# MarSaKi/VLN-BEVBert

Hardware: AMD Instinct MI355X
Metric: pretrain_samples_per_sec (higher is better)
Workload: dtype bf16+fp32-residual

## Files before the change

include/bevbert_hip.h:

```cpp
#ifndef BEVBERT_HIP_H
#define BEVBERT_HIP_H

#include <stdint.h>

#ifdef __cplusplus
extern "C" {
#endif

typedef struct ihipStream_t* hipStream_t;

#define BEVBERT_F32 0
#define BEVBERT_BF16 1
#define BEVBERT_F16 2

const char* bevbert_last_error(void);
int bevbert_version(void);
int bevbert_hip_error_reset(void);
const char* bevbert_arch(void);
const char* bevbert_attn_last_path(int backward);
const char* bevbert_attn_plan(int B, int nh, int Lq, int Lk, int dtype, int impl, int has_key_mask, int has_bias,
                              float drop_p, int has_bits, int bits_ready, int want_dbias, int ncu, int backward);

int bevbert_bev_lift_bin(const float* depths, const float* T_c2w, const float* T_w2c, const float* S_w2c,
                         const float* pix_scale, int B, int V, int hw, float depth_scale, int dim, float res,
                         float y_clip, int* cell, int* order, int* cell_start, hipStream_t stream);
int bevbert_bev_bin_points(const float* points, const uint8_t* drop_mask, int B, int P, int dim, float res,
                           float y_clip, int* cell, int* order, int* cell_start, hipStream_t stream);
int bevbert_bev_splat_mean(const void* feat, int feat_dtype, const int* order, const int* cell_start, void* out,
                           int out_dtype, int B, int P, int K, int C, const uint8_t* sem_ids, const double* sem_dense,
                           int S, uint8_t* out_sem, uint8_t* out_sem_mask, const int* sample_rows, int rows_per_sample,
                           hipStream_t stream);

int bevbert_attn_fwd(const void* q, const void* k, const void* v, void* o, float* lse, const float* key_mask,
                     const float* bias, const int64_t* strides, int B, int nh, int Lq, int Lk, int head_dim,
                     float scale, int dtype, int impl, float drop_p, uint64_t seed, uint64_t offset,
                     uint64_t* drop_bits, int bits_ready, hipStream_t stream);
int bevbert_attn_bwd(const void* q, const void* k, const void* v, const void* o, const void* dout, const float* lse,
                     float* delta_ws, void* dq, void* dk, void* dv, float* dbias, const float* key_mask,
                     const float* bias, const int64_t* strides, int B, int nh, int Lq, int Lk, int head_dim,
                     float scale, int dtype, int impl, float drop_p, uint64_t seed, uint64_t offset,
                     const uint64_t* drop_bits, hipStream_t stream);
int64_t bevbert_attn_drop_bits_words(int B, int nh, int Lq, int Lk);
int bevbert_attn_drop_bits(uint64_t* drop_bits, int B, int nh, int Lq, int Lk, float drop_p, uint64_t seed,
                           uint64_t offset, hipStream_t stream);
int bevbert_attn_bits_ahead(int Lq, int Lk, int has_bias);

int bevbert_bias_dropout_residual_layernorm_fwd(const void* x, const float* bias, const void* residual,
                                                const float* gamma, const float* beta, void* y, void* z_out,
                                                float* mean, float* rstd, int rows, int H, float eps, int dtype,
                                                float drop_p, uint64_t seed, uint64_t offset, hipStream_t stream);
int bevbert_layernorm_post_fwd(const void* x, const float* bias, const float* gamma, const float* beta,
                               const void* post1, const void* post2, void* y, void* z_out, float* mean, float* rstd,
                               int rows, int H, float eps, int dtype, hipStream_t stream);
int bevbert_layernorm_bwd(const void* dy, const void* z, const float* mean, const float* rstd, const float* gamma,
// ... 204 lines not shown
```

vln_bevbert_amd/csrc/capi.hip:

```cpp
#include <stdarg.h>

#include "attn_common.h"

static thread_local char g_err[512] = "";

void bb_set_error(const char* fmt, ...) {
  va_list ap;
  va_start(ap, fmt);
  vsnprintf(g_err, sizeof(g_err), fmt, ap);
  va_end(ap);
}

BEVBERT_API const char* bevbert_last_error(void) { return g_err; }
BEVBERT_API int bevbert_hip_error_reset(void) {
  int n = 0;
  while (hipGetLastError() != hipSuccess && n < 16) ++n;
  return n;
}

BEVBERT_API int bevbert_zero(void* p, int64_t bytes, hipStream_t stream) {
  BB_REQUIRE(p != nullptr && bytes >= 0, "zero: null pointer or negative size");
  if (bytes == 0) return BB_OK;
  hipError_t e = hipMemsetAsync(p, 0, (size_t)bytes, stream);
  if (e != hipSuccess) {
    bb_set_error("zero: hipMemsetAsync failed: %s", hipGetErrorString(e));
    return BB_ELAUNCH;
  }
  return BB_OK;
}

BEVBERT_API int bevbert_version(void) { return 201; }

static const uint32_t* g_step_salt = nullptr;
const uint32_t* bb_step_salt() { return g_step_salt; }
BEVBERT_API int bevbert_set_step_salt(const void* device_word) {
  g_step_salt = static_cast<const uint32_t*>(device_word);
  return BB_OK;
}
BEVBERT_API const char* bevbert_arch(void) { return "gfx950"; }

int attn_simple_fwd(const AttnArgs& a, int dtype, hipStream_t st);
int attn_simple_bwd(const AttnArgs& a, int dtype, hipStream_t st);
int attn_delta(const AttnArgs& a, float* delta, int dtype, hipStream_t st);
int attn_mfma_fwd(const AttnArgs& a, hipStream_t st);
int attn_mfma_bwd(const AttnArgs& a, hipStream_t st);
int attn_mfma_bwd1(const AttnArgs& a, hipStream_t st);
bool attn_mfma_bwd1_supported(const AttnArgs& a);
int attn_fwd2(const AttnArgs& a, hipStream_t st);
bool attn_fwd2_supported(const AttnArgs& a);
int attn_drop_bits(const AttnArgs& a, uint64_t* bits_f, uint64_t* bits_b, uint32_t* bits_l, hipStream_t st);
int attn_fwd4(const AttnArgs& a, const uint32_t* bits_l, hipStream_t st);
bool attn_fwd4_supported(const AttnArgs& a, int ncu, bool forced);
int attn_fwd4_workgroups();
int attn_bwd2(const AttnArgs& a, hipStream_t st);
// ... 256 lines not shown
```

vln_bevbert_amd/csrc/splat.hip:

```cpp
#include "common.h"

#define MAX_CELLS 1024
#define MAX_POINTS 24576

struct LiftArgs {
  const float* depths;
  const float* T_c2w;
  const float* T_w2c;
  const float* S_w2c;
  const float* pix;
  const float* points;
  const uint8_t* pmask;
  int V, hw;
  float depth_scale;
  int P, dim;
  float res, half, y_clip;
  int* cell;
  int* order;
  int* cell_start;
};

__device__ __forceinline__ int cell_of(float ex, float ey, float ez, bool dropped, int dim, float res, float half,
                                       float y_clip) {
  const float fx = rintf(__fadd_rn(__fdiv_rn(ex, res), half));
  const float fz = rintf(__fadd_rn(__fdiv_rn(ez, res), half));
  const float fd = (float)dim;
  const bool outside = (fx >= fd) | (fz >= fd) | (fx < 0.f) | (fz < 0.f);
  if (dropped | outside | (ey > y_clip)) return -1;
  return dim * (int)fz + (int)fx;
}

template <int MODE>
__global__ __launch_bounds__(256) void bev_bin_sort_kernel(LiftArgs a) {
  __shared__ short s_cell[MAX_POINTS];
  __shared__ int s_cnt[MAX_CELLS + 1];
  const int b = blockIdx.x, tid = threadIdx.x;
  const int K = a.dim * a.dim;
  for (int c = tid; c <= K; c += 256) s_cnt[c] = 0;
  __syncthreads();

  for (int p = tid; p < a.P; p += 256) {
    int cid;
    if (MODE == 0) {
      const int hw2 = a.hw * a.hw;
      const int v = p / hw2, r = (p - v * hw2) / a.hw, u = p % a.hw;
      const float z = __fmul_rn(a.depths[(size_t)b * a.P + p], a.depth_scale);
      const float x = __fmul_rn(z, a.pix[u]);
      const float y = __fmul_rn(z, a.pix[r]);
      const float* T = a.T_c2w + ((size_t)b * a.V + v) * 16;
      float w[3];
#pragma unroll
      for (int i = 0; i < 3; ++i)
        w[i] = __fadd_rn(__fadd_rn(__fadd_rn(__fmul_rn(T[i * 4 + 0], x), __fmul_rn(T[i * 4 + 1], y)),
                                   __fmul_rn(T[i * 4 + 2], z)),
                         T[i * 4 + 3]);
      const float* S = a.S_w2c + (size_t)b * 3;
      const float p0 = __fsub_rn(w[0], S[0]), p1 = __fsub_rn(w[1], S[1]), p2 = __fsub_rn(w[2], S[2]);
      const float* R = a.T_w2c + (size_t)b * 16;
      float e[3];
#pragma unroll
      for (int i = 0; i < 3; ++i)
        e[i] = __fadd_rn(__fadd_rn(__fadd_rn(__fmul_rn(R[i * 4 + 0], p0), __fmul_rn(R[i * 4 + 1], p1)),
                                   __fmul_rn(R[i * 4 + 2], p2)),
                         R[i * 4 + 3]);
      cid = cell_of(e[0], e[1], e[2], z == 0.f, a.dim, a.res, a.half, a.y_clip);
    } else {
      const float* q = a.points + ((size_t)b * a.P + p) * 3;
      cid = cell_of(q[0], q[1], q[2], a.pmask[(size_t)b * a.P + p] != 0, a.dim, a.res, a.half, a.y_clip);
    }
    s_cell[p] = (short)cid;
    a.cell[(size_t)b * a.P + p] = cid;
    if (cid >= 0) atomicAdd(&s_cnt[cid], 1);
  }
  __syncthreads();

  if (tid < 64) {
    const int per = (K + 63) / 64;
    const int c0 = tid * per;
    int sum = 0;
    for (int i = 0; i < per; ++i)
      if (c0 + i < K) sum += s_cnt[c0 + i];
    int incl = sum;
#pragma unroll
    for (int o = 1; o < 64; o <<= 1) {
      int t = __shfl_up(incl, o, 64);
      if (tid >= o) incl += t;
    }
    int run = incl - sum;
    for (int i = 0; i < per; ++i)
      if (c0 + i < K) {
        const int n = s_cnt[c0 + i];
        s_cnt[c0 + i] = run;
        run += n;
      }
    if (tid == 63) s_cnt[K] = incl;
  }
  __syncthreads();
  for (int c = tid; c <= K; c += 256) a.cell_start[(size_t)b * (K + 1) + c] = s_cnt[c];

  __shared__ int s_wbase[4][MAX_CELLS + 1];
  const int lane = tid & 63, wv = tid >> 6;
  for (int c = tid; c < 4 * (MAX_CELLS + 1); c += 256) (&s_wbase[0][0])[c] = 0;
  __syncthreads();
  const int per_wave = ((a.P + 255) / 256) * 64;
  const int pw0 = wv * per_wave;
  for (int p = pw0 + lane; p < pw0 + per_wave && p < a.P; p += 64) {
    const int cid = s_cell[p];
    if (cid >= 0) atomicAdd(&s_wbase[wv][cid], 1);
  }
  __syncthreads();
  for (int c = tid; c < K; c += 256) {
    int base = s_cnt[c];
#pragma unroll
    for (int w = 0; w < 4; ++w) {
      const int n = s_wbase[w][c];
      s_wbase[w][c] = base;
      base += n;
    }
  }
  __syncthreads();
  int* dst = a.order + (size_t)b * a.P;
  const unsigned long long lt = lane == 0 ? 0ull : (~0ull >> (64 - lane));
  for (int p0 = pw0; p0 < pw0 + per_wave && p0 < a.P; p0 += 64) {
    const int p = p0 + lane;
    const int cid = p < a.P ? (int)s_cell[p] : -1;
    unsigned long long todo = __ballot(cid >= 0);
    while (todo) {
      const int leader = __builtin_ctzll(todo);
      const int c0 = __shfl(cid, leader, 64);
      const unsigned long long same = __ballot(cid == c0);
      const int base = s_wbase[wv][c0];
      if (cid == c0) dst[base + __builtin_popcountll(same & lt)] = p;
      if (lane == leader) s_wbase[wv][c0] = base + __builtin_popcountll(same);
      todo &= ~same;
    }
  }
}

template <typename TI, typename TO>
__global__ __launch_bounds__(256) void bev_splat_mean_kernel(const TI* __restrict__ feat, const int* __restrict__ order,
                                                             const int* __restrict__ cell_start, TO* __restrict__ out,
                                                             int P, int K, int C,
                                                             const uint8_t* __restrict__ sem_ids,
                                                             const double* __restrict__ sem_dense,
                                                             int S, uint8_t* __restrict__ out_sem,
                                                             uint8_t* __restrict__ out_sem_mask,
                                                             const int* __restrict__ sample_rows,
                                                             int R) {
  const int cellg = blockIdx.x;
  const int b = cellg / K, cell = cellg - b * K;
  const int P0 = P / R;
  const int* rows = sample_rows != nullptr ? sample_rows + (size_t)b * R : nullptr;
  auto src_point = [&](int p) -> size_t {
    if (rows == nullptr) return (size_t)b * P + p;
    if (R == 1) return (size_t)rows[0] * P0 + p;
    const int r = p / P0;
    return (size_t)rows[r] * P0 + (p - r * P0);
  };
  const int s0 = cell_start[(size_t)b * (K + 1) + cell];
  const int n = cell_start[(size_t)b * (K + 1) + cell + 1] - s0;
  const int* ord = order + (size_t)b * P + s0;
  const float inv_denominator = (float)(n > 1 ? n : 1);

  for (int c4 = threadIdx.x; c4 * 4 < C; c4 += blockDim.x) {
    float4 acc = make_float4(0.f, 0.f, 0.f, 0.f);
    int i = 0;
    for (; i + 4 <= n; i += 4) {
      const int p0 = ord[i], p1 = ord[i + 1], p2 = ord[i + 2], p3 = ord[i + 3];
      const float4 v0 = ld4<TI>(feat + src_point(p0) * C + c4 * 4);
      const float4 v1 = ld4<TI>(feat + src_point(p1) * C + c4 * 4);
      const float4 v2 = ld4<TI>(feat + src_point(p2) * C + c4 * 4);
      const float4 v3 = ld4<TI>(feat + src_point(p3) * C + c4 * 4);
      acc.x = __fadd_rn(__fadd_rn(__fadd_rn(__fadd_rn(acc.x, v0.x), v1.x), v2.x), v3.x);
      acc.y = __fadd_rn(__fadd_rn(__fadd_rn(__fadd_rn(acc.y, v0.y), v1.y), v2.y), v3.y);
      acc.z = __fadd_rn(__fadd_rn(__fadd_rn(__fadd_rn(acc.z, v0.z), v1.z), v2.z), v3.z);
      acc.w = __fadd_rn(__fadd_rn(__fadd_rn(__fadd_rn(acc.w, v0.w), v1.w), v2.w), v3.w);
    }
    for (; i < n; ++i) {
      const float4 v = ld4<TI>(feat + src_point(ord[i]) * C + c4 * 4);
      acc.x = __fadd_rn(acc.x, v.x); acc.y = __fadd_rn(acc.y, v.y);
      acc.z = __fadd_rn(acc.z, v.z); acc.w = __fadd_rn(acc.w, v.w);
    }
    acc.x = __fdiv_rn(acc.x, inv_denominator); acc.y = __fdiv_rn(acc.y, inv_denominator);
    acc.z = __fdiv_rn(acc.z, inv_denominator); acc.w = __fdiv_rn(acc.w, inv_denominator);
    st4<TO>(out + (size_t)cellg * C + c4 * 4, acc);
  }

  if (out_sem != nullptr) {
    int any = 0;
    for (int c = threadIdx.x; c < S; c += blockDim.x) {
      uint8_t flag = 0;
      if (sem_ids != nullptr) {
        for (int i = 0; i < n; ++i) flag |= (uint8_t)(sem_ids[src_point(ord[i])] == (uint8_t)c);
      } else {
        const double* sb = sem_dense + (size_t)b * P * S;
        double acc = 0.0;
        for (int i = 0; i < n; ++i) acc += sb[(size_t)ord[i] * S + c];
        flag = (uint8_t)(acc / (double)(n > 1 ? n : 1) > 0.0);
      }
      out_sem[(size_t)cellg * S + c] = flag;
      any |= flag;
    }
    any = __syncthreads_or(any);
    if (threadIdx.x == 0) out_sem_mask[cellg] = (uint8_t)(any != 0);
  }
}

BEVBERT_API int bevbert_bev_lift_bin(const float* depths, const float* T_c2w, const float* T_w2c, const float* S_w2c,
                                     const float* pix_scale, int B, int V, int hw, float depth_scale, int dim,
                                     float res, float y_clip, int* cell, int* order, int* cell_start,
                                     hipStream_t stream) {
  const int P = V * hw * hw;
  BB_REQUIRE(B > 0 && P > 0 && P <= MAX_POINTS, "bev_lift_bin: P=%d out of range (max %d)", P, MAX_POINTS);
  BB_REQUIRE(dim > 0 && dim * dim <= MAX_CELLS, "bev_lift_bin: dim=%d too large", dim);
  LiftArgs a;
  memset(&a, 0, sizeof(a));
  a.depths = depths; a.T_c2w = T_c2w; a.T_w2c = T_w2c; a.S_w2c = S_w2c; a.pix = pix_scale;
  a.V = V; a.hw = hw; a.depth_scale = depth_scale; a.P = P; a.dim = dim; a.res = res;
  a.half = (float)(dim - 1) / 2.0f; a.y_clip = y_clip;
  a.cell = cell; a.order = order; a.cell_start = cell_start;
  hipLaunchKernelGGL(bev_bin_sort_kernel<0>, dim3(B), dim3(256), 0, stream, a);
  BB_CHECK_LAUNCH("bev_lift_bin");
  return BB_OK;
}

BEVBERT_API int bevbert_bev_bin_points(const float* points, const uint8_t* drop_mask, int B, int P, int dim, float res,
                                       float y_clip, int* cell, int* order, int* cell_start, hipStream_t stream) {
  BB_REQUIRE(B > 0 && P > 0 && P <= MAX_POINTS, "bev_bin_points: P=%d out of range (max %d)", P, MAX_POINTS);
  BB_REQUIRE(dim > 0 && dim * dim <= MAX_CELLS, "bev_bin_points: dim=%d too large", dim);
  LiftArgs a;
  memset(&a, 0, sizeof(a));
  a.points = points; a.pmask = drop_mask; a.P = P; a.dim = dim; a.res = res;
  a.half = (float)(dim - 1) / 2.0f; a.y_clip = y_clip;
  a.cell = cell; a.order = order; a.cell_start = cell_start;
  hipLaunchKernelGGL(bev_bin_sort_kernel<1>, dim3(B), dim3(256), 0, stream, a);
  BB_CHECK_LAUNCH("bev_bin_points");
  return BB_OK;
}

template <typename TI, typename TO>
static int launch_splat(const void* feat, const int* order, const int* cell_start, void* out, int B, int P, int K,
                        int C, const uint8_t* sem_ids, const double* sem_dense, int S, uint8_t* out_sem,
                        uint8_t* out_sem_mask, const int* sample_rows, int R, hipStream_t stream) {
  const int threads = (C / 4 >= 192) ? 192 : ((C / 4 + 63) / 64) * 64;
  hipLaunchKernelGGL((bev_splat_mean_kernel<TI, TO>), dim3(B * K), dim3(threads < 64 ? 64 : threads), 0, stream,
                     (const TI*)feat, order, cell_start, (TO*)out, P, K, C, sem_ids, sem_dense, S, out_sem,
                     out_sem_mask, sample_rows, R);
  BB_CHECK_LAUNCH("bev_splat_mean");
  return BB_OK;
}

BEVBERT_API int bevbert_bev_splat_mean(const void* feat, int feat_dtype, const int* order, const int* cell_start,
                                       void* out, int out_dtype, int B, int P, int K, int C, const uint8_t* sem_ids,
                                       const double* sem_dense, int S, uint8_t* out_sem, uint8_t* out_sem_mask,
                                       const int* sample_rows, int rows_per_sample, hipStream_t stream) {
  BB_REQUIRE(C % 4 == 0, "bev_splat_mean: C=%d must be a multiple of 4", C);
  const int R = rows_per_sample < 1 ? 1 : rows_per_sample;
  BB_REQUIRE(R == 1 || sample_rows != nullptr, "bev_splat_mean: rows_per_sample=%d needs sample_rows", R);
  BB_REQUIRE(P % R == 0, "bev_splat_mean: P=%d is not a multiple of rows_per_sample=%d", P, R);
  BB_REQUIRE(sample_rows == nullptr || sem_dense == nullptr,
             "bev_splat_mean: sample_rows indexes feat / sem_ids stores; dense semantics are per batch");
  BB_REQUIRE(out_sem == nullptr || (sem_ids != nullptr) != (sem_dense != nullptr),
             "bev_splat_mean: exactly one of sem_ids / sem_dense when semantics are requested");
#define GO(TI, TO) \
  return launch_splat<TI, TO>(feat, order, cell_start, out, B, P, K, C, sem_ids, sem_dense, S, out_sem, out_sem_mask, sample_rows, R, stream)
  if (feat_dtype == BB_F32 && out_dtype == BB_F32) GO(float, float);
  if (feat_dtype == BB_F32 && out_dtype == BB_BF16) GO(float, bf16_raw);
  if (feat_dtype == BB_BF16 && out_dtype == BB_F32) GO(bf16_raw, float);
  if (feat_dtype == BB_BF16 && out_dtype == BB_BF16) GO(bf16_raw, bf16_raw);
  if (feat_dtype == BB_F16 && out_dtype == BB_F32) GO(_Float16, float);
  if (feat_dtype == BB_F16 && out_dtype == BB_BF16) GO(_Float16, bf16_raw);
  if (feat_dtype == BB_F16 && out_dtype == BB_F16) GO(_Float16, _Float16);
#undef GO
  bb_set_error("bev_splat_mean: unsupported dtype pair (%d -> %d)", feat_dtype, out_dtype);
  return BB_EUNSUPPORTED;
}
```

vln_bevbert_amd/lib.py:

```python
import ctypes
import os
import re
import subprocess

import torch

_HERE = os.path.dirname(os.path.abspath(__file__))
LIB_PATH = os.path.join(_HERE, "libbevbert_hip.so")
CSRC = os.path.join(_HERE, "csrc")
EXTRA_FLAGS = {"attn_fwd4.hip": ["-fno-slp-vectorize"]}
SOURCES = ["splat.hip", "rowops.hip", "attn_simple.hip", "attn_f32.hip", "attn_mfma.hip", "attn_bwd1.hip", "attn_fwd2.hip", "attn_fwd4.hip", "attn_bwd2.hip", "attn_bwd3.hip", "attn_small.hip", "attn_short.hip", "smallk.hip", "sap_loss.hip", "graph_nav.hip", "nav_expert.hip", "waypoint.hip", "gemm.hip", "capi.hip"]
HEADER = os.path.join(os.path.dirname(_HERE), "include", "bevbert_hip.h")

F32, BF16, F16 = 0, 1, 2
_DT = {torch.float32: F32, torch.bfloat16: BF16, torch.float16: F16}


class BevBertHipError(RuntimeError):
    pass


def dtype_code(t):
    try:
        return _DT[t.dtype if torch.is_tensor(t) else t]
# ... 21 lines not shown
    def run(cmd):
        if verbose:
            print(" ".join(cmd), flush=True)
        subprocess.run(cmd, check=True, cwd=CSRC)

    with ThreadPoolExecutor(max_workers=min(8, max(1, len(jobs)))) as ex:
        list(ex.map(run, jobs))
    run([hipcc, "--offload-arch=gfx950", "-shared", "-fPIC", "-o", LIB_PATH] + objs + ["-lhipblaslt"])
    return LIB_PATH


def header_symbols():
    with open(HEADER) as f:
        return sorted(set(re.findall(r"\b(bevbert_\w+)\s*\(", f.read())))


_lib = None
_P, _I, _I64, _U64, _F = ctypes.c_void_p, ctypes.c_int, ctypes.c_int64, ctypes.c_uint64, ctypes.c_float

_PROTOS = {
    "bevbert_bev_lift_bin": [_P, _P, _P, _P, _P, _I, _I, _I, _F, _I, _F, _F, _P, _P, _P, _P],
    "bevbert_bev_bin_points": [_P, _P, _I, _I, _I, _F, _F, _P, _P, _P, _P],
    "bevbert_bev_splat_mean": [_P, _I, _P, _P, _P, _I, _I, _I, _I, _I, _P, _P, _I, _P, _P, _P, _I, _P],
    "bevbert_attn_fwd": [_P, _P, _P, _P, _P, _P, _P, _P, _I, _I, _I, _I, _I, _F, _I, _I, _F, _U64, _U64, _P, _I, _P],
    "bevbert_attn_drop_bits": [_P, _I, _I, _I, _I, _F, _U64, _U64, _P],
    "bevbert_attn_bwd": [_P, _P, _P, _P, _P, _P, _P, _P, _P, _P, _P, _P, _P, _P, _I, _I, _I, _I, _I, _F, _I, _I, _F,
                         _U64, _U64, _P, _P],
    "bevbert_bias_dropout_residual_layernorm_fwd": [_P, _P, _P, _P, _P, _P, _P, _P, _P, _I, _I, _F, _I, _F, _U64,
                                                    _U64, _P],
    "bevbert_layernorm_post_fwd": [_P, _P, _P, _P, _P, _P, _P, _P, _P, _P, _I, _I, _F, _I, _P],
    "bevbert_layernorm_bwd": [_P, _P, _P, _P, _P, _P, _P, _P, _P, _P, _P, _I, _I, _I, _F, _U64, _U64, _I, _P],
    "bevbert_layernorm_res32_fwd": [_P, _P, _P, _I, _P, _P, _P, _P, _P, _P, _P, _I, _I, _F, _F, _U64, _U64, _P],
    "bevbert_layernorm_res32_bwd": [_P, _P, _P, _P, _P, _P, _P, _P, _P, _P, _P, _P, _I, _I, _F, _U64, _U64, _I, _I, _P],
    "bevbert_colsum_any": [_P, _P, _I, _I, _I, _I, _P],
    "bevbert_sem_select": [_P, _P, _I, _I, _I, _P, _P, _P, _P],
    "bevbert_bce_rows_fwd": [_P, _P, _P, _P, _I, _I, _I, _P],
    "bevbert_bce_rows_bwd": [_P, _P, _P, _P, _P, _I, _I, _I, _P],
    "bevbert_weighted_mean_fwd": [_P, _P, _P, _F, _I, _P, _P],
    "bevbert_weighted_mean_bwd": [_P, _P, _P, _F, _I, _P, _P],
    "bevbert_layernorm_bwd_add": [_P, _P, _P, _P, _P, _P, _P, _P, _P, _P, _P, _P, _I, _I, _I, _F, _U64, _U64, _I, _P],
    "bevbert_embed_sum_layernorm_fwd": [_P, _P, _P, _P, _P, _P, _P, _P, _P, _P, _I, _I, _I, _F, _I, _F, _U64, _U64, _P],
    "bevbert_embedding_grad": [_P, _P, _P, _I, _I, _I, _I, _P],
    "bevbert_rows_gather": [_P, _P, _P, _I, _I, _I, _P],
    "bevbert_graph_bias_fwd": [_P, _P, _P, _P, _I64, _P],
    "bevbert_graph_bias_bwd": [_P, _P, _I, _I, _I, _I, _P, _P, _P, _P],
    "bevbert_smallk_linear_layernorm_fwd": [_P] * 11 + [_I, _I, _I, _F, _I, _P],
# ... 131 lines not shown
```

vln_bevbert_amd/ops_rowops.py:

```python
import math

import torch

from . import lib
from .lib import dtype_code, ptr, stream
from .ops_core import RT, _compute, _f32, _mark_touched, _sink, call
from .ops_reduce import ReduceQueue, WgradStream, _on_launch_stream, _partial_rows


def embedding_grad_small(ids, d, sink, table_rows):
    rows, H = d.shape
    per = 64
    while (rows + per - 1) // per * table_rows > 4096:
        per *= 2
    slices = (rows + per - 1) // per
    part = RT.scratch.alloc(slices * table_rows * H * 4, d.device)
    call("bevbert_embedding_grad_sliced", ptr(ids), ptr(d), part, rows, H, table_rows, per, dtype_code(d), stream())
    ReduceQueue.add(part, slices, 1, table_rows * H, (sink.data_ptr(), None, None))


class _BiasDropResLN(torch.autograd.Function):
    @staticmethod
    def forward(ctx, x, bias, residual, gamma, beta, eps, drop_p, inplace_z, post1=None, post2=None, return_z=False):
        assert x.is_contiguous() and x.dim() >= 2
# ... 670 lines not shown
    cell_start = torch.empty(B, dim * dim + 1, dtype=torch.int32, device=dev)
    f = lambda t: t.contiguous().float()
    d, a, b_, c_ = f(depths), f(T_c2w), f(T_w2c), f(S_w2c)
    call("bevbert_bev_lift_bin", ptr(d), ptr(a), ptr(b_), ptr(c_), ptr(pix), B, V, hw, float(depth_scale), dim,
         float(res), float(y_clip), ptr(cell), ptr(order), ptr(cell_start), stream())
    return cell, order, cell_start


@torch.no_grad()
def bev_bin_points(points, drop_mask, dim, res, y_clip=0.5):
    B, P = points.shape[0], points.shape[1]
    dev = points.device
    cell = torch.empty(B, P, dtype=torch.int32, device=dev)
    order = torch.zeros(B, P, dtype=torch.int32, device=dev)
    cell_start = torch.empty(B, dim * dim + 1, dtype=torch.int32, device=dev)
    pts = points.contiguous().float()
    dm = drop_mask.contiguous().to(torch.uint8)
    call("bevbert_bev_bin_points", ptr(pts), ptr(dm), B, P, dim, float(res), float(y_clip), ptr(cell), ptr(order),
         ptr(cell_start), stream())
    return cell, order, cell_start


@torch.no_grad()
def bev_splat_mean(feat, order, cell_start, K, out_dtype=None, sems=None, n_classes=40, rows=None):
    C = feat.shape[-1]
    B, P = order.shape
    R = 1 if rows is None or rows.dim() == 1 else rows.shape[1]
    assert P == R * feat.shape[1] if rows is not None else feat.shape[:2] == (B, P)
    assert feat.is_contiguous() if rows is not None else True
    feat = feat.contiguous()
    out_dtype = out_dtype or (feat.dtype if feat.dtype != torch.float16 else torch.float32)
    out = torch.empty(B, K, C, dtype=out_dtype, device=feat.device)
    sem_ids = sem_dense = out_sem = out_mask = None
    S = n_classes
    if sems is not None:
        if sems.dim() == 2:
            sem_ids = sems.contiguous().to(torch.uint8)
            assert sem_ids.shape[1] * R == P and (rows is not None or sem_ids.shape[0] == B)
        else:
            sem_dense = sems.contiguous().to(torch.float64)
            S = sems.shape[-1]
        out_sem = torch.empty(B, K, S, dtype=torch.uint8, device=feat.device)
        out_mask = torch.empty(B, K, dtype=torch.bool, device=feat.device)
    call("bevbert_bev_splat_mean", ptr(feat), dtype_code(feat), ptr(order), ptr(cell_start), ptr(out),
         dtype_code(out_dtype), B, P, K, C, ptr(sem_ids), ptr(sem_dense), S, ptr(out_sem), ptr(out_mask),
         ptr(rows.contiguous() if rows is not None else None), R, stream())
    return out, out_sem, out_mask


def dropout_keep_mask(n, drop_p, seed, offset, device):
    out = torch.empty(n, dtype=torch.uint8, device=device)
    call("bevbert_dropout_keep_mask", ptr(out), n, float(drop_p), int(seed), int(offset), stream())
    return out.bool()
```

vln_bevbert_amd/pretrain_cmt.py:

```python

import numpy as np
import torch
import torch.nn.functional as F
from torch import nn

from . import ops
from .config import BevBertConfig
from .vilmodel import BertOnlyMLMHead, GlocalTextPathCMT, ensure_arena, finalize, from_pretrained, gen_seq_masks

BEV_DIM = 21
BEV_RES = 0.5


def bevpos_polar(dim, device):
    c = torch.linspace(0.5, dim - 0.5, dim, dtype=torch.float32)
    ry, rx = torch.meshgrid(c, c, indexing="ij")
    ry = -(ry - dim / 2)
    rx = rx - dim / 2
    dis = (ry ** 2 + rx ** 2) ** 0.5
    cos, sin = rx / dis, ry / dis
    cos[dis == 0] = 0
    sin[dis == 0] = 0
    return torch.stack([cos, sin, dis / (dim / 2)], -1).reshape(dim * dim, 3).to(device)

# ... 110 lines not shown

    @classmethod
    def from_pretrained(cls, pretrained_model_name_or_path=None, config=None, state_dict=None, **kwargs):
        return from_pretrained(cls, pretrained_model_name_or_path, config, state_dict)

    def finalize(self, device, compute_dtype=torch.float32, residual=None):
        return finalize(self, device, compute_dtype, residual)

    feat_dropout = property(lambda self: self.drop_env.p, lambda self, v: setattr(self.drop_env, "p", v))

    def set_dropout(self, p):
        for m in self.modules():
            if isinstance(m, nn.Dropout):
                m.p = p
            if hasattr(m, "attn_drop_p"):
                m.attn_drop_p = p

    def _projector(self, device):
        if self._proj is None or self._proj[0].device != device:
            cfg = self.config
            self._proj = (ops.pixel_scale(cfg.grid_hw, device), bevpos_polar(cfg.bev_dim, device))
        return self._proj

    def lift_splat(self, batch):
        cfg = self.config
        T_c2w, T_w2c, S_w2c = batch.pop("T_c2w"), batch.pop("T_w2c"), batch.pop("S_w2c")
        bev_gpos_fts = batch.pop("bev_gpos_fts")
        store, rows = batch.pop("grid_store", None), batch.pop("grid_rows", None)
        if store is not None:
            feat, sem_in = store.rgbs, (store.sems if cfg.sem_classes > 0 else None)
            depths = store.depths.index_select(0, rows.long())
        else:
            rgbs, depths, sems = batch.pop("rgbs"), batch.pop("depths"), batch.pop("sems", None)
            feat = rgbs.reshape(rgbs.shape[0], -1, rgbs.shape[-1])
            sem_in = None if sems is None else (sems if sems.dim() == 2 else sems.reshape(feat.shape[0], feat.shape[1], -1))
        B = depths.shape[0]
        dev = depths.device
        dim, K = cfg.bev_dim, cfg.bev_dim * cfg.bev_dim
        pix, polar = self._projector(dev)
        cell, order, cell_start = ops.bev_lift_bin(depths, T_c2w, T_w2c, S_w2c, pix, dim, cfg.bev_res)
        cd = ops._compute(self.bert.local_encoder.bev_fts_embeddings[0].weight).dtype
        bev_fts, bev_sems, bev_sem_masks = ops.bev_splat_mean(feat, order, cell_start, K, out_dtype=cd, sems=sem_in,
                                                              n_classes=cfg.sem_classes, rows=rows)
        bev_pos_fts = torch.cat([bev_gpos_fts.expand(-1, K, -1), polar[None].expand(B, -1, -1)], dim=-1)
        batch.update({
            "bev_fts": bev_fts,
            "bev_masks": self._all_ones(B, K, dev),
            "bev_pos_fts": bev_pos_fts,
            "bev_sems": bev_sems,
            "bev_sem_masks": None if bev_sem_masks is None else bev_sem_masks.bool(),
            "_bev_masks_all_ones": True,
            "_bev_cell": cell,
        })
        return batch

    def _all_ones(self, B, K, dev):
        c = self.__dict__.setdefault("_ones_cache", {})
        t = c.get((B, K, dev))
        if t is None:
            t = c[(B, K, dev)] = torch.ones(B, K, dtype=torch.bool, device=dev)
        return t

    def drop_feats(self, batch):
        cd = ops._compute(self.bert.local_encoder.bev_fts_embeddings[0].weight).dtype
        for k in ("traj_view_img_fts", "traj_obj_img_fts", "bev_fts"):
            if batch.get(k) is not None:
                batch[k] = ops.dropout(batch[k], self.feat_dropout, self.training, out_dtype=cd)
        return batch

    _CMT_KEYS = ["txt_ids", "txt_lens", "traj_view_img_fts", "traj_obj_img_fts", "traj_loc_fts", "traj_nav_types",
                 "traj_step_lens", "traj_vp_view_lens", "traj_vp_obj_lens", "traj_vpids", "traj_cand_vpids",
                 "gmap_lens", "gmap_step_ids", "gmap_pos_fts", "gmap_pair_dists", "gmap_vpids",
                 "bev_fts", "bev_pos_fts", "bev_masks", "bev_nav_masks"]

    def _cmt_args(self, b):
        args = [b.get(k) for k in self._CMT_KEYS]
        if b.get("_bev_masks_all_ones"):
            args[18] = True
        return args

    def loss_mean(self, batch, task):
        return self.forward(batch, task, compute_loss="mean")

    def forward(self, batch, task, compute_loss=True):
        if not any(task.startswith(t) for t in ("mlm", "mrc", "sap", "og", "sem", "masksem")):
            raise ValueError("invalid task")
        ensure_arena(self)
        batch = dict(batch)
        self.lift_splat(batch)
        self.drop_feats(batch)
        if task.startswith("mlm"):
            return self.forward_mlm(batch, compute_loss)
        if task.startswith("sap"):
            return self.forward_sap(batch, compute_loss)
        if task.startswith("mrc"):
            return self.forward_mrc(batch, compute_loss)
        if task.startswith("og"):
            return self.forward_og(batch, compute_loss)
        if task.startswith("masksem"):
            return self.forward_masksem(batch, compute_loss)
        return self.forward_sem(batch, compute_loss)

    def _host_kw(self, b):
        kw = {"view_lens_host": b.get("traj_vp_view_lens_cpu"), "obj_lens_host": b.get("traj_vp_obj_lens_cpu"),
              "gmap_csr": b.get("gmap_csr")}
        if getattr(self.config, "depth_feat_size", 0) > 0:
            kw["traj_view_dep_fts"] = b["traj_view_dep_fts"]
        return kw

    def forward_mrc(self, b, compute_loss):
        _, _, obj_embeds, _ = self.bert(*self._cmt_args(b), return_gmap_embeds=False, **self._host_kw(b))
        sel = b["vp_obj_mrc_masks"]
        host = b.get("vp_obj_mrc_masks_cpu")
# ... 151 lines not shown
```

Measured before the change: 3576.

## Fuse BEV feature dropout into splat-mean and restructure bin-sort and splat kernels

Adds a dropout-fused variant of the BEV splat-mean kernel so bev_fts is dropped inside the splat epilogue rather than in a separate dropout pass. It also rewrites bin-sort to use 1024 threads, ballot-based per-wave counting instead of shared atomics, and camera matrices staged in shared memory. The splat kernel moves to one wave per cell with broadcast row indices and batched row loads. This removes a kernel launch and a full read/write of bev_fts and reduces atomic contention, but the dropout mask stream differs from the standalone dropout op.

Measured after the change: 3560. Within noise of the previous version (-0.4%).

```diff
diff --git a/include/bevbert_hip.h b/include/bevbert_hip.h
--- a/include/bevbert_hip.h
+++ b/include/bevbert_hip.h
@@ -30,6 +30,11 @@
                            int out_dtype, int B, int P, int K, int C, const uint8_t* sem_ids, const double* sem_dense,
                            int S, uint8_t* out_sem, uint8_t* out_sem_mask, const int* sample_rows, int rows_per_sample,
                            hipStream_t stream);
+int bevbert_bev_splat_mean_drop(const void* feat, int feat_dtype, const int* order, const int* cell_start, void* out,
+                                int out_dtype, int B, int P, int K, int C, const uint8_t* sem_ids,
+                                const double* sem_dense, int S, uint8_t* out_sem, uint8_t* out_sem_mask,
+                                const int* sample_rows, int rows_per_sample, float drop_p, uint64_t seed,
+                                uint64_t offset, hipStream_t stream);
 
 int bevbert_attn_fwd(const void* q, const void* k, const void* v, void* o, float* lse, const float* key_mask,
                      const float* bias, const int64_t* strides, int B, int nh, int Lq, int Lk, int head_dim,
diff --git a/vln_bevbert_amd/csrc/capi.hip b/vln_bevbert_amd/csrc/capi.hip
--- a/vln_bevbert_amd/csrc/capi.hip
+++ b/vln_bevbert_amd/csrc/capi.hip
@@ -29,7 +29,7 @@
   return BB_OK;
 }
 
-BEVBERT_API int bevbert_version(void) { return 201; }
+BEVBERT_API int bevbert_version(void) { return 202; }
 
 static const uint32_t* g_step_salt = nullptr;
 const uint32_t* bb_step_salt() { return g_step_salt; }
diff --git a/vln_bevbert_amd/csrc/splat.hip b/vln_bevbert_amd/csrc/splat.hip
--- a/vln_bevbert_amd/csrc/splat.hip
+++ b/vln_bevbert_amd/csrc/splat.hip
@@ -30,124 +30,157 @@
   return dim * (int)fz + (int)fx;
 }
 
+__device__ __forceinline__ int lift_cell(const LiftArgs& a, int b, int p, const float* T_all, const float* R,
+                                         const float* S, const float* pix) {
+  const int hw2 = a.hw * a.hw;
+  const int v = p / hw2, r = (p - v * hw2) / a.hw, u = p % a.hw;
+  const float z = __fmul_rn(a.depths[(size_t)b * a.P + p], a.depth_scale);
+  const float x = __fmul_rn(z, pix[u]);
+  const float y = __fmul_rn(z, pix[r]);
+  const float* T = T_all + (size_t)v * 16;
+  float w[3];
+#pragma unroll
+  for (int i = 0; i < 3; ++i)
+    w[i] = __fadd_rn(__fadd_rn(__fadd_rn(__fmul_rn(T[i * 4 + 0], x), __fmul_rn(T[i * 4 + 1], y)),
+                               __fmul_rn(T[i * 4 + 2], z)),
+                     T[i * 4 + 3]);
+  const float p0 = __fsub_rn(w[0], S[0]), p1 = __fsub_rn(w[1], S[1]), p2 = __fsub_rn(w[2], S[2]);
+  float e[3];
+#pragma unroll
+  for (int i = 0; i < 3; ++i)
+    e[i] = __fadd_rn(__fadd_rn(__fadd_rn(__fmul_rn(R[i * 4 + 0], p0), __fmul_rn(R[i * 4 + 1], p1)),
+                               __fmul_rn(R[i * 4 + 2], p2)),
+                     R[i * 4 + 3]);
+  return cell_of(e[0], e[1], e[2], z == 0.f, a.dim, a.res, a.half, a.y_clip);
+}
+
+__device__ __forceinline__ unsigned long long same_cell_lanes(int cid, int nbits) {
+  unsigned long long same = __ballot(cid >= 0);
+  for (int bit = 0; bit < nbits; ++bit) {
+    const bool set = (cid >> bit) & 1;
+    const unsigned long long m = __ballot(set);
+    same &= set ? m : ~m;
+  }
+  return same;
+}
+
+#define BIN_THREADS 1024
+#define BIN_WAVES (BIN_THREADS / 64)
+#define BIN_STAGE_VIEWS 128
+#define BIN_STAGE_HW 256
+
 template <int MODE>
-__global__ __launch_bounds__(256) void bev_bin_sort_kernel(LiftArgs a) {
+__global__ __launch_bounds__(BIN_THREADS) void bev_bin_sort_kernel(LiftArgs a) {
   __shared__ short s_cell[MAX_POINTS];
-  __shared__ int s_cnt[MAX_CELLS + 1];
+  __shared__ int s_wbase[BIN_WAVES][MAX_CELLS + 1];
+  __shared__ int s_wtot[BIN_WAVES];
+  __shared__ float s_T[BIN_STAGE_VIEWS * 16 + 16 + 4];
+  __shared__ float s_pix[BIN_STAGE_HW];
   const int b = blockIdx.x, tid = threadIdx.x;
+  const int lane = tid & 63, wv = tid >> 6;
   const int K = a.dim * a.dim;
-  for (int c = tid; c <= K; c += 256) s_cnt[c] = 0;
+  const int nbits = K > 1 ? 32 - __builtin_clz(K - 1) : 0;
+  const bool staged = MODE == 0 && a.V <= BIN_STAGE_VIEWS && a.hw <= BIN_STAGE_HW;
+  for (int w = 0; w < BIN_WAVES; ++w)
+    if (tid < K) s_wbase[w][tid] = 0;
+  if (staged) {
+    float* s_R = s_T + BIN_STAGE_VIEWS * 16;
+    float* s_S = s_R + 16;
+    for (int i = tid; i < a.V * 16; i += BIN_THREADS) s_T[i] = a.T_c2w[(size_t)b * a.V * 16 + i];
+    if (tid < 16) s_R[tid] = a.T_w2c[(size_t)b * 16 + tid];
+    if (tid < 3) s_S[tid] = a.S_w2c[(size_t)b * 3 + tid];
+    if (tid < a.hw) s_pix[tid] = a.pix[tid];
+  }
   __syncthreads();
 
-  for (int p = tid; p < a.P; p += 256) {
-    int cid;
-    if (MODE == 0) {
-      const int hw2 = a.hw * a.hw;
-      const int v = p / hw2, r = (p - v * hw2) / a.hw, u = p % a.hw;
-      const float z = __fmul_rn(a.depths[(size_t)b * a.P + p], a.depth_scale);
-      const float x = __fmul_rn(z, a.pix[u]);
-      const float y = __fmul_rn(z, a.pix[r]);
-      const float* T = a.T_c2w + ((size_t)b * a.V + v) * 16;
-      float w[3];
-#pragma unroll
-      for (int i = 0; i < 3; ++i)
-        w[i] = __fadd_rn(__fadd_rn(__fadd_rn(__fmul_rn(T[i * 4 + 0], x), __fmul_rn(T[i * 4 + 1], y)),
-                                   __fmul_rn(T[i * 4 + 2], z)),
-                         T[i * 4 + 3]);
-      const float* S = a.S_w2c + (size_t)b * 3;
-      const float p0 = __fsub_rn(w[0], S[0]), p1 = __fsub_rn(w[1], S[1]), p2 = __fsub_rn(w[2], S[2]);
-      const float* R = a.T_w2c + (size_t)b * 16;
-      float e[3];
-#pragma unroll
-      for (int i = 0; i < 3; ++i)
-        e[i] = __fadd_rn(__fadd_rn(__fadd_rn(__fmul_rn(R[i * 4 + 0], p0), __fmul_rn(R[i * 4 + 1], p1)),
-                                   __fmul_rn(R[i * 4 + 2], p2)),
-                         R[i * 4 + 3]);
-      cid = cell_of(e[0], e[1], e[2], z == 0.f, a.dim, a.res, a.half, a.y_clip);
-    } else {
-      const float* q = a.points + ((size_t)b * a.P + p) * 3;
-      cid = cell_of(q[0], q[1], q[2], a.pmask[(size_t)b * a.P + p] != 0, a.dim, a.res, a.half, a.y_clip);
-    }
-    s_cell[p] = (short)cid;
-    a.cell[(size_t)b * a.P + p] = cid;
-    if (cid >= 0) atomicAdd(&s_cnt[cid], 1);
+  const int per_wave = ((a.P + BIN_THREADS - 1) / BIN_THREADS) * 64;
+  const int pw0 = wv * per_wave;
+  const int pw1 = min(pw0 + per_wave, a.P);
+  for (int p0 = pw0; p0 < pw1; p0 += 64) {
+    const int p = p0 + lane;
+    int cid = -1;
+    if (p < pw1) {
+      if (MODE == 0) {
+        if (staged)
+          cid = lift_cell(a, b, p, s_T, s_T + BIN_STAGE_VIEWS * 16, s_T + BIN_STAGE_VIEWS * 16 + 16, s_pix);
+        else
+          cid = lift_cell(a, b, p, a.T_c2w + (size_t)b * a.V * 16, a.T_w2c + (size_t)b * 16, a.S_w2c + (size_t)b * 3,
+                          a.pix);
+      } else {
+        const float* q = a.points + ((size_t)b * a.P + p) * 3;
+        cid = cell_of(q[0], q[1], q[2], a.pmask[(size_t)b * a.P + p] != 0, a.dim, a.res, a.half, a.y_clip);
+      }
+      s_cell[p] = (short)cid;
+      a.cell[(size_t)b * a.P + p] = cid;
+    }
+    const unsigned long long same = same_cell_lanes(cid, nbits);
+    if (cid >= 0 && lane == __builtin_ctzll(same)) s_wbase[wv][cid] += __builtin_popcountll(same);
   }
   __syncthreads();
 
-  if (tid < 64) {
-    const int per = (K + 63) / 64;
-    const int c0 = tid * per;
-    int sum = 0;
-    for (int i = 0; i < per; ++i)
-      if (c0 + i < K) sum += s_cnt[c0 + i];
-    int incl = sum;
-#pragma unroll
-    for (int o = 1; o < 64; o <<= 1) {
-      int t = __shfl_up(incl, o, 64);
-      if (tid >= o) incl += t;
-    }
-    int run = incl - sum;
-    for (int i = 0; i < per; ++i)
-      if (c0 + i < K) {
-        const int n = s_cnt[c0 + i];
-        s_cnt[c0 + i] = run;
-        run += n;
-      }
-    if (tid == 63) s_cnt[K] = incl;
-  }
+  int cnt = 0;
+  if (tid < K)
+    for (int w = 0; w < BIN_WAVES; ++w) cnt += s_wbase[w][tid];
+  int incl = cnt;
+#pragma unroll
+  for (int o = 1; o < 64; o <<= 1) {
+    const int t = __shfl_up(incl, o, 64);
+    if (lane >= o) incl += t;
+  }
+  if (lane == 63) s_wtot[wv] = incl;
   __syncthreads();
-  for (int c = tid; c <= K; c += 256) a.cell_start[(size_t)b * (K + 1) + c] = s_cnt[c];
-
-  __shared__ int s_wbase[4][MAX_CELLS + 1];
-  const int lane = tid & 63, wv = tid >> 6;
-  for (int c = tid; c < 4 * (MAX_CELLS + 1); c += 256) (&s_wbase[0][0])[c] = 0;
+  int before = 0, total = 0;
+  for (int w = 0; w < BIN_WAVES; ++w) {
+    const int t = s_wtot[w];
+    if (w < wv) before += t;
+    total += t;
+  }
+  if (tid < K) {
+    int base = before + incl - cnt;
+    a.cell_start[(size_t)b * (K + 1) + tid] = base;
+    for (int w = 0; w < BIN_WAVES; ++w) {
+      const int n = s_wbase[w][tid];
+      s_wbase[w][tid] = base;
+      base += n;
+    }
+  }
+  if (tid == 0) a.cell_start[(size_t)b * (K + 1) + K] = total;
   __syncthreads();
-  const int per_wave = ((a.P + 255) / 256) * 64;
-  const int pw0 = wv * per_wave;
-  for (int p = pw0 + lane; p < pw0 + per_wave && p < a.P; p += 64) {
-    const int cid = s_cell[p];
-    if (cid >= 0) atomicAdd(&s_wbase[wv][cid], 1);
-  }
-  __syncthreads();
-  for (int c = tid; c < K; c += 256) {
-    int base = s_cnt[c];
-#pragma unroll
-    for (int w = 0; w < 4; ++w) {
-      const int n = s_wbase[w][c];
-      s_wbase[w][c] = base;
-      base += n;
-    }
-  }
-  __syncthreads();
+
   int* dst = a.order + (size_t)b * a.P;
   const unsigned long long lt = lane == 0 ? 0ull : (~0ull >> (64 - lane));
-  for (int p0 = pw0; p0 < pw0 + per_wave && p0 < a.P; p0 += 64) {
+  for (int p0 = pw0; p0 < pw1; p0 += 64) {
     const int p = p0 + lane;
-    const int cid = p < a.P ? (int)s_cell[p] : -1;
-    unsigned long long todo = __ballot(cid >= 0);
-    while (todo) {
-      const int leader = __builtin_ctzll(todo);
-      const int c0 = __shfl(cid, leader, 64);
-      const unsigned long long same = __ballot(cid == c0);
-      const int base = s_wbase[wv][c0];
-      if (cid == c0) dst[base + __builtin_popcountll(same & lt)] = p;
-      if (lane == leader) s_wbase[wv][c0] = base + __builtin_popcountll(same);
-      todo &= ~same;
-    }
-  }
-}
-
-template <typename TI, typename TO>
+    const int cid = p < pw1 ? (int)s_cell[p] : -1;
+    const unsigned long long same = same_cell_lanes(cid, nbits);
+    if (cid >= 0) {
+      const int base = s_wbase[wv][cid];
+      dst[base + __builtin_popcountll(same & lt)] = p;
+      if (lane == __builtin_ctzll(same)) s_wbase[wv][cid] = base + __builtin_popcountll(same);
+    }
+  }
+}
+
+template <typename TO> __device__ __forceinline__ float round_through(float v);
+template <> __device__ __forceinline__ float round_through<float>(float v) { return v; }
+template <> __device__ __forceinline__ float round_through<bf16_raw>(float v) { return bf16_to_f32(f32_to_bf16(v)); }
+template <> __device__ __forceinline__ float round_through<_Float16>(float v) { return (float)(_Float16)v; }
+
+#define SPLAT_ROWS 8
+template <typename TI, typename TO, int NCH>
 __global__ __launch_bounds__(256) void bev_splat_mean_kernel(const TI* __restrict__ feat, const int* __restrict__ order,
                                                              const int* __restrict__ cell_start, TO* __restrict__ out,
-                                                             int P, int K, int C,
+                                                             int ncells, int P, int K, int C,
                                                              const uint8_t* __restrict__ sem_ids,
                                                              const double* __restrict__ sem_dense,
                                                              int S, uint8_t* __restrict__ out_sem,
                                                              uint8_t* __restrict__ out_sem_mask,
                                                              const int* __restrict__ sample_rows,
-                                                             int R) {
-  const int cellg = blockIdx.x;
+                                                             int R, int drop, float keep_scale, uint32_t thr,
+                                                             uint32_t key, const uint32_t* __restrict__ salt) {
+  const int lane = threadIdx.x & 63;
+  const int cellg = blockIdx.x * 4 + __builtin_amdgcn_readfirstlane(threadIdx.x >> 6);
+  if (cellg >= ncells) return;
   const int b = cellg / K, cell = cellg - b * K;
   const int P0 = P / R;
   const int* rows = sample_rows != nullptr ? sample_rows + (size_t)b * R : nullptr;
@@ -161,48 +194,90 @@
   const int n = cell_start[(size_t)b * (K + 1) + cell + 1] - s0;
   const int* ord = order + (size_t)b * P + s0;
   const float inv_denominator = (float)(n > 1 ? n : 1);
-
-  for (int c4 = threadIdx.x; c4 * 4 < C; c4 += blockDim.x) {
-    float4 acc = make_float4(0.f, 0.f, 0.f, 0.f);
-    int i = 0;
-    for (; i + 4 <= n; i += 4) {
-      const int p0 = ord[i], p1 = ord[i + 1], p2 = ord[i + 2], p3 = ord[i + 3];
-      const float4 v0 = ld4<TI>(feat + src_point(p0) * C + c4 * 4);
-      const float4 v1 = ld4<TI>(feat + src_point(p1) * C + c4 * 4);
-      const float4 v2 = ld4<TI>(feat + src_point(p2) * C + c4 * 4);
-      const float4 v3 = ld4<TI>(feat + src_point(p3) * C + c4 * 4);
-      acc.x = __fadd_rn(__fadd_rn(__fadd_rn(__fadd_rn(acc.x, v0.x), v1.x), v2.x), v3.x);
-      acc.y = __fadd_rn(__fadd_rn(__fadd_rn(__fadd_rn(acc.y, v0.y), v1.y), v2.y), v3.y);
-      acc.z = __fadd_rn(__fadd_rn(__fadd_rn(__fadd_rn(acc.z, v0.z), v1.z), v2.z), v3.z);
-      acc.w = __fadd_rn(__fadd_rn(__fadd_rn(__fadd_rn(acc.w, v0.w), v1.w), v2.w), v3.w);
-    }
-    for (; i < n; ++i) {
-      const float4 v = ld4<TI>(feat + src_point(ord[i]) * C + c4 * 4);
-      acc.x = __fadd_rn(acc.x, v.x); acc.y = __fadd_rn(acc.y, v.y);
-      acc.z = __fadd_rn(acc.z, v.z); acc.w = __fadd_rn(acc.w, v.w);
-    }
-    acc.x = __fdiv_rn(acc.x, inv_denominator); acc.y = __fdiv_rn(acc.y, inv_denominator);
-    acc.z = __fdiv_rn(acc.z, inv_denominator); acc.w = __fdiv_rn(acc.w, inv_denominator);
-    st4<TO>(out + (size_t)cellg * C + c4 * 4, acc);
+  if (drop) key = bb_salted(key, salt);
+
+  for (int cb = 0; cb * 4 < C; cb += 64 * NCH) {
+    float4 acc[NCH];
+#pragma unroll
+    for (int j = 0; j < NCH; ++j) acc[j] = make_float4(0.f, 0.f, 0.f, 0.f);
+    for (int i0 = 0; i0 < n; i0 += 64) {
+      const int cnt = min(64, n - i0);
+      size_t my = 0;
+      if (lane < cnt) my = src_point(ord[i0 + lane]);
+      const uint32_t my_lo = (uint32_t)my, my_hi = (uint32_t)(my >> 32);
+      for (int i = 0; i < cnt; i += SPLAT_ROWS) {
+        float4 v[SPLAT_ROWS][NCH];
+#pragma unroll
+        for (int k = 0; k < SPLAT_ROWS; ++k) {
+#pragma unroll
+          for (int j = 0; j < NCH; ++j) v[k][j] = make_float4(0.f, 0.f, 0.f, 0.f);
+          if (i + k < cnt) {
+            const size_t row = ((size_t)__builtin_amdgcn_readlane(my_hi, i + k) << 32) |
+                               (size_t)__builtin_amdgcn_readlane(my_lo, i + k);
+            const TI* rp = feat + row * C;
+#pragma unroll
+            for (int j = 0; j < NCH; ++j) {
+              const int c4 = cb + j * 64 + lane;
+              if (c4 * 4 < C) v[k][j] = ld4<TI>(rp + c4 * 4);
+            }
+          }
+        }
+#pragma unroll
+        for (int k = 0; k < SPLAT_ROWS; ++k)
+#pragma unroll
+          for (int j = 0; j < NCH; ++j) {
+            acc[j].x = __fadd_rn(acc[j].x, v[k][j].x); acc[j].y = __fadd_rn(acc[j].y, v[k][j].y);
+            acc[j].z = __fadd_rn(acc[j].z, v[k][j].z); acc[j].w = __fadd_rn(acc[j].w, v[k][j].w);
+          }
+      }
+    }
+#pragma unroll
+    for (int j = 0; j < NCH; ++j) {
+      const int c4 = cb + j * 64 + lane;
+      if (c4 * 4 >= C) continue;
+      float4 m;
+      m.x = __fdiv_rn(acc[j].x, inv_denominator); m.y = __fdiv_rn(acc[j].y, inv_denominator);
+      m.z = __fdiv_rn(acc[j].z, inv_denominator); m.w = __fdiv_rn(acc[j].w, inv_denominator);
+      if (drop) {
+        const uint32_t pr = (uint32_t)((((size_t)cellg * C) / 4 + c4) * 2);
+        const uint32_t b0 = bb_pair_bits(key, pr), b1 = bb_pair_bits(key, pr + 1);
+        m.x = bb_keep_lo(b0, thr) ? __fmul_rn(round_through<TO>(m.x), keep_scale) : 0.f;
+        m.y = bb_keep_hi(b0, thr) ? __fmul_rn(round_through<TO>(m.y), keep_scale) : 0.f;
+        m.z = bb_keep_lo(b1, thr) ? __fmul_rn(round_through<TO>(m.z), keep_scale) : 0.f;
+        m.w = bb_keep_hi(b1, thr) ? __fmul_rn(round_through<TO>(m.w), keep_scale) : 0.f;
+      }
+      st4<TO>(out + (size_t)cellg * C + c4 * 4, m);
+    }
   }
 
   if (out_sem != nullptr) {
     int any = 0;
-    for (int c = threadIdx.x; c < S; c += blockDim.x) {
+    for (int cs = 0; cs < S; cs += 64) {
+      const int c = cs + lane;
       uint8_t flag = 0;
-      if (sem_ids != nullptr) {
-        for (int i = 0; i < n; ++i) flag |= (uint8_t)(sem_ids[src_point(ord[i])] == (uint8_t)c);
-      } else {
-        const double* sb = sem_dense + (size_t)b * P * S;
-        double acc = 0.0;
-        for (int i = 0; i < n; ++i) acc += sb[(size_t)ord[i] * S + c];
-        flag = (uint8_t)(acc / (double)(n > 1 ? n : 1) > 0.0);
-      }
-      out_sem[(size_t)cellg * S + c] = flag;
-      any |= flag;
-    }
-    any = __syncthreads_or(any);
-    if (threadIdx.x == 0) out_sem_mask[cellg] = (uint8_t)(any != 0);
+      double dacc = 0.0;
+      for (int i0 = 0; i0 < n; i0 += 64) {
+        const int cnt = min(64, n - i0);
+        int pl = 0, sid = -1;
+        if (lane < cnt) {
+          pl = ord[i0 + lane];
+          if (sem_ids != nullptr) sid = sem_ids[src_point(pl)];
+        }
+        if (sem_ids != nullptr) {
+          for (int i = 0; i < cnt; ++i) flag |= (uint8_t)(__builtin_amdgcn_readlane(sid, i) == (int)(uint8_t)c);
+        } else if (c < S) {
+          const double* sb = sem_dense + (size_t)b * P * S;
+          for (int i = 0; i < cnt; ++i) dacc += sb[(size_t)__builtin_amdgcn_readlane(pl, i) * S + c];
+        }
+      }
+      if (sem_ids == nullptr) flag = (uint8_t)(dacc / (double)(n > 1 ? n : 1) > 0.0);
+      if (c < S) {
+        out_sem[(size_t)cellg * S + c] = flag;
+        any |= flag;
+      }
+    }
+    const bool any_class = __ballot(any != 0) != 0ull;
+    if (lane == 0) out_sem_mask[cellg] = (uint8_t)any_class;
   }
 }
 
@@ -219,7 +294,7 @@
   a.V = V; a.hw = hw; a.depth_scale = depth_scale; a.P = P; a.dim = dim; a.res = res;
   a.half = (float)(dim - 1) / 2.0f; a.y_clip = y_clip;
   a.cell = cell; a.order = order; a.cell_start = cell_start;
-  hipLaunchKernelGGL(bev_bin_sort_kernel<0>, dim3(B), dim3(256), 0, stream, a);
+  hipLaunchKernelGGL(bev_bin_sort_kernel<0>, dim3(B), dim3(BIN_THREADS), 0, stream, a);
   BB_CHECK_LAUNCH("bev_lift_bin");
   return BB_OK;
 }
@@ -233,27 +308,40 @@
   a.points = points; a.pmask = drop_mask; a.P = P; a.dim = dim; a.res = res;
   a.half = (float)(dim - 1) / 2.0f; a.y_clip = y_clip;
   a.cell = cell; a.order = order; a.cell_start = cell_start;
-  hipLaunchKernelGGL(bev_bin_sort_kernel<1>, dim3(B), dim3(256), 0, stream, a);
+  hipLaunchKernelGGL(bev_bin_sort_kernel<1>, dim3(B), dim3(BIN_THREADS), 0, stream, a);
   BB_CHECK_LAUNCH("bev_bin_points");
   return BB_OK;
 }
+
+struct SplatDrop {
+  int drop;
+  float keep_scale;
+  uint32_t thr, key;
+};
 
 template <typename TI, typename TO>
 static int launch_splat(const void* feat, const int* order, const int* cell_start, void* out, int B, int P, int K,
                         int C, const uint8_t* sem_ids, const double* sem_dense, int S, uint8_t* out_sem,
-                        uint8_t* out_sem_mask, const int* sample_rows, int R, hipStream_t stream) {
-  const int threads = (C / 4 >= 192) ? 192 : ((C / 4 + 63) / 64) * 64;
-  hipLaunchKernelGGL((bev_splat_mean_kernel<TI, TO>), dim3(B * K), dim3(threads < 64 ? 64 : threads), 0, stream,
-                     (const TI*)feat, order, cell_start, (TO*)out, P, K, C, sem_ids, sem_dense, S, out_sem,
-                     out_sem_mask, sample_rows, R);
+                        uint8_t* out_sem_mask, const int* sample_rows, int R, SplatDrop d, hipStream_t stream) {
+  const int ncells = B * K;
+  const uint32_t* salt = d.drop ? bb_step_salt() : nullptr;
+#define SPLAT_GO(NCH)                                                                                                 \
+  hipLaunchKernelGGL((bev_splat_mean_kernel<TI, TO, NCH>), dim3((ncells + 3) / 4), dim3(256), 0, stream,              \
+                     (const TI*)feat, order, cell_start, (TO*)out, ncells, P, K, C, sem_ids, sem_dense, S, out_sem,   \
+                     out_sem_mask, sample_rows, R, d.drop, d.keep_scale, d.thr, d.key, salt)
+  if (C <= 256) SPLAT_GO(1);
+  else if (C <= 768) SPLAT_GO(3);
+  else SPLAT_GO(4);
+#undef SPLAT_GO
   BB_CHECK_LAUNCH("bev_splat_mean");
   return BB_OK;
 }
 
-BEVBERT_API int bevbert_bev_splat_mean(const void* feat, int feat_dtype, const int* order, const int* cell_start,
-                                       void* out, int out_dtype, int B, int P, int K, int C, const uint8_t* sem_ids,
-                                       const double* sem_dense, int S, uint8_t* out_sem, uint8_t* out_sem_mask,
-                                       const int* sample_rows, int rows_per_sample, hipStream_t stream) {
+static int splat_dispatch(const void* feat, int feat_dtype, const int* order, const int* cell_start, void* out,
+                          int out_dtype, int B, int P, int K, int C, const uint8_t* sem_ids, const double* sem_dense,
+                          int S, uint8_t* out_sem, uint8_t* out_sem_mask, const int* sample_rows, int rows_per_sample,
+                          SplatDrop d, hipStream_t stream) {
+  BB_REQUIRE(B > 0 && K > 0, "bev_splat_mean: B=%d K=%d", B, K);
   BB_REQUIRE(C % 4 == 0, "bev_splat_mean: C=%d must be a multiple of 4", C);
   const int R = rows_per_sample < 1 ? 1 : rows_per_sample;
   BB_REQUIRE(R == 1 || sample_rows != nullptr, "bev_splat_mean: rows_per_sample=%d needs sample_rows", R);
@@ -263,7 +351,7 @@
   BB_REQUIRE(out_sem == nullptr || (sem_ids != nullptr) != (sem_dense != nullptr),
              "bev_splat_mean: exactly one of sem_ids / sem_dense when semantics are requested");
 #define GO(TI, TO) \
-  return launch_splat<TI, TO>(feat, order, cell_start, out, B, P, K, C, sem_ids, sem_dense, S, out_sem, out_sem_mask, sample_rows, R, stream)
+  return launch_splat<TI, TO>(feat, order, cell_start, out, B, P, K, C, sem_ids, sem_dense, S, out_sem, out_sem_mask, sample_rows, R, d, stream)
   if (feat_dtype == BB_F32 && out_dtype == BB_F32) GO(float, float);
   if (feat_dtype == BB_F32 && out_dtype == BB_BF16) GO(float, bf16_raw);
   if (feat_dtype == BB_BF16 && out_dtype == BB_F32) GO(bf16_raw, float);
@@ -275,3 +363,30 @@
   bb_set_error("bev_splat_mean: unsupported dtype pair (%d -> %d)", feat_dtype, out_dtype);
   return BB_EUNSUPPORTED;
 }
+
+BEVBERT_API int bevbert_bev_splat_mean(const void* feat, int feat_dtype, const int* order, const int* cell_start,
+                                       void* out, int out_dtype, int B, int P, int K, int C, const uint8_t* sem_ids,
+                                       const double* sem_dense, int S, uint8_t* out_sem, uint8_t* out_sem_mask,
+                                       const int* sample_rows, int rows_per_sample, hipStream_t stream) {
+  SplatDrop d;
+  memset(&d, 0, sizeof(d));
+  return splat_dispatch(feat, feat_dtype, order, cell_start, out, out_dtype, B, P, K, C, sem_ids, sem_dense, S, out_sem,
+                        out_sem_mask, sample_rows, rows_per_sample, d, stream);
+}
+
+BEVBERT_API int bevbert_bev_splat_mean_drop(const void* feat, int feat_dtype, const int* order, const int* cell_start,
+                                            void* out, int out_dtype, int B, int P, int K, int C,
+                                            const uint8_t* sem_ids, const double* sem_dense, int S, uint8_t* out_sem,
+                                            uint8_t* out_sem_mask, const int* sample_rows, int rows_per_sample,
+                                            float drop_p, uint64_t seed, uint64_t offset, hipStream_t stream) {
+  BB_REQUIRE(drop_p >= 0.f && drop_p < 1.f, "bev_splat_mean_drop: p=%f out of range", drop_p);
+  BB_REQUIRE((int64_t)B * K * C < ((int64_t)1 << 32), "bev_splat_mean_drop: %ld elements, must be below 2^32",
+             (long)((int64_t)B * K * C));
+  SplatDrop d;
+  d.drop = 1;
+  d.keep_scale = 1.0f / (1.0f - drop_p);
+  d.thr = bb_drop_threshold(drop_p);
+  d.key = bb_site_key(seed, offset);
+  return splat_dispatch(feat, feat_dtype, order, cell_start, out, out_dtype, B, P, K, C, sem_ids, sem_dense, S, out_sem,
+                        out_sem_mask, sample_rows, rows_per_sample, d, stream);
+}
diff --git a/vln_bevbert_amd/lib.py b/vln_bevbert_amd/lib.py
--- a/vln_bevbert_amd/lib.py
+++ b/vln_bevbert_amd/lib.py
@@ -67,6 +67,7 @@
     "bevbert_bev_lift_bin": [_P, _P, _P, _P, _P, _I, _I, _I, _F, _I, _F, _F, _P, _P, _P, _P],
     "bevbert_bev_bin_points": [_P, _P, _I, _I, _I, _F, _F, _P, _P, _P, _P],
     "bevbert_bev_splat_mean": [_P, _I, _P, _P, _P, _I, _I, _I, _I, _I, _P, _P, _I, _P, _P, _P, _I, _P],
+    "bevbert_bev_splat_mean_drop": [_P, _I, _P, _P, _P, _I, _I, _I, _I, _I, _P, _P, _I, _P, _P, _P, _I, _F, _U64, _U64, _P],
     "bevbert_attn_fwd": [_P, _P, _P, _P, _P, _P, _P, _P, _I, _I, _I, _I, _I, _F, _I, _I, _F, _U64, _U64, _P, _I, _P],
     "bevbert_attn_drop_bits": [_P, _I, _I, _I, _I, _F, _U64, _U64, _P],
     "bevbert_attn_bwd": [_P, _P, _P, _P, _P, _P, _P, _P, _P, _P, _P, _P, _P, _P, _I, _I, _I, _I, _I, _F, _I, _I, _F,
diff --git a/vln_bevbert_amd/ops_rowops.py b/vln_bevbert_amd/ops_rowops.py
--- a/vln_bevbert_amd/ops_rowops.py
+++ b/vln_bevbert_amd/ops_rowops.py
@@ -716,7 +716,7 @@
 
 
 @torch.no_grad()
-def bev_splat_mean(feat, order, cell_start, K, out_dtype=None, sems=None, n_classes=40, rows=None):
+def bev_splat_mean(feat, order, cell_start, K, out_dtype=None, sems=None, n_classes=40, rows=None, drop_p=0.0):
     C = feat.shape[-1]
     B, P = order.shape
     R = 1 if rows is None or rows.dim() == 1 else rows.shape[1]
@@ -736,9 +736,13 @@
             S = sems.shape[-1]
         out_sem = torch.empty(B, K, S, dtype=torch.uint8, device=feat.device)
         out_mask = torch.empty(B, K, dtype=torch.bool, device=feat.device)
-    call("bevbert_bev_splat_mean", ptr(feat), dtype_code(feat), ptr(order), ptr(cell_start), ptr(out),
-         dtype_code(out_dtype), B, P, K, C, ptr(sem_ids), ptr(sem_dense), S, ptr(out_sem), ptr(out_mask),
-         ptr(rows.contiguous() if rows is not None else None), R, stream())
+    args = (ptr(feat), dtype_code(feat), ptr(order), ptr(cell_start), ptr(out), dtype_code(out_dtype), B, P, K, C,
+            ptr(sem_ids), ptr(sem_dense), S, ptr(out_sem), ptr(out_mask),
+            ptr(rows.contiguous() if rows is not None else None), R)
+    if drop_p > 0.0:
+        call("bevbert_bev_splat_mean_drop", *args, float(drop_p), RT.seed, RT.next_offset(out.numel()), stream())
+    else:
+        call("bevbert_bev_splat_mean", *args, stream())
     return out, out_sem, out_mask
 
 
diff --git a/vln_bevbert_amd/pretrain_cmt.py b/vln_bevbert_amd/pretrain_cmt.py
--- a/vln_bevbert_amd/pretrain_cmt.py
+++ b/vln_bevbert_amd/pretrain_cmt.py
@@ -156,7 +156,7 @@
             self._proj = (ops.pixel_scale(cfg.grid_hw, device), bevpos_polar(cfg.bev_dim, device))
         return self._proj
 
-    def lift_splat(self, batch):
+    def lift_splat(self, batch, drop_p=0.0):
         cfg = self.config
         T_c2w, T_w2c, S_w2c = batch.pop("T_c2w"), batch.pop("T_w2c"), batch.pop("S_w2c")
         bev_gpos_fts = batch.pop("bev_gpos_fts")
@@ -175,7 +175,7 @@
         cell, order, cell_start = ops.bev_lift_bin(depths, T_c2w, T_w2c, S_w2c, pix, dim, cfg.bev_res)
         cd = ops._compute(self.bert.local_encoder.bev_fts_embeddings[0].weight).dtype
         bev_fts, bev_sems, bev_sem_masks = ops.bev_splat_mean(feat, order, cell_start, K, out_dtype=cd, sems=sem_in,
-                                                              n_classes=cfg.sem_classes, rows=rows)
+                                                              n_classes=cfg.sem_classes, rows=rows, drop_p=drop_p)
         bev_pos_fts = torch.cat([bev_gpos_fts.expand(-1, K, -1), polar[None].expand(B, -1, -1)], dim=-1)
         batch.update({
             "bev_fts": bev_fts,
@@ -195,9 +195,9 @@
             t = c[(B, K, dev)] = torch.ones(B, K, dtype=torch.bool, device=dev)
         return t
 
-    def drop_feats(self, batch):
+    def drop_feats(self, batch, keys=("traj_view_img_fts", "traj_obj_img_fts", "bev_fts")):
         cd = ops._compute(self.bert.local_encoder.bev_fts_embeddings[0].weight).dtype
-        for k in ("traj_view_img_fts", "traj_obj_img_fts", "bev_fts"):
+        for k in keys:
             if batch.get(k) is not None:
                 batch[k] = ops.dropout(batch[k], self.feat_dropout, self.training, out_dtype=cd)
         return batch
@@ -221,8 +221,12 @@
             raise ValueError("invalid task")
         ensure_arena(self)
         batch = dict(batch)
-        self.lift_splat(batch)
-        self.drop_feats(batch)
+        if self.training and self.feat_dropout > 0.0 and _os.environ.get("BEVBERT_FUSE_BEV_DROPOUT", "1") == "1":
+            self.drop_feats(batch, keys=("traj_view_img_fts", "traj_obj_img_fts"))
+            self.lift_splat(batch, drop_p=self.feat_dropout)
+        else:
+            self.lift_splat(batch)
+            self.drop_feats(batch)
         if task.startswith("mlm"):
             return self.forward_mlm(batch, compute_loss)
         if task.startswith("sap"):
```
